# kursawe/OpticalFlow

Hardware: AMD Instinct MI355X
Metric: frame-pairs/sec (higher is better)
Workload: dtype f64; 1 GPU; 1024x1024x256 synthetic translating texture (seed 1), speed_alpha=1, remodelling_alpha=1e4, rtol=1e-06, all 255 pairs solved to the stopping rule; frames_per_gpu=256, pairs_in_flight=255, levels=9, coarse_stencils=float8, vcycle_vectors=coarse_float32, w_cycle_level=1, w_cycle_visits=3, warm_start_stride=3, allgather=False, gather_chunks=1, converged=True

## Files before the change

### opticalflow_amd/csrc/vof_device.hpp

```cpp
#pragma once
#include <hip/hip_runtime.h>
#include <stdint.h>
#include <type_traits>

namespace vof {

constexpr int BX = 64;
constexpr int BY = 4;
constexpr int NT = BX * BY;

struct PairScalars {
    double rho, alpha, omega, beta;
    double bnorm2, rnorm2;
    double tol2;
    int iterations;
    int converged;
    int breakdown;
    int halfstep;
};

struct PairParam {
    double alpha, beta;
    int frame;
    int out;
// ... 151 lines not shown
        blk[1] += scale * (s * P * k.Dy / 2);
        blk[2] += scale * (-s * P / 2);
        blk[3] += scale * (s * P * k.Dy / 2);
        blk[4] += scale * alpha;
        blk[6] += scale * (s * P / 2);
        blk[8] += scale * beta;
    } else if (oi == 0) {
        T s = (T)oj;
        blk[0] += scale * alpha;
        blk[1] += scale * (s * P * k.Dx / 2);
        blk[3] += scale * (s * P * k.Dx / 2);
        blk[4] += scale * (P * (s * k.Dy + P) + alpha);
        blk[5] += scale * (-s * P / 2);
        blk[7] += scale * (s * P / 2);
        blk[8] += scale * beta;
    } else {
        T s = (T)(oi * oj);
        blk[1] += scale * (s * P * P / 4);
        blk[3] += scale * (s * P * P / 4);
    }
}

__host__ __device__ constexpr unsigned raw_block_mask(int oi, int oj) {
    return (oi == 0 && oj == 0) ? 0x1DBu
         : (oj == 0)            ? 0x15Fu
         : (oi == 0)            ? 0x1BBu
                                : 0x00Au;
}

template <typename T, typename KT>
__device__ __forceinline__ void folded_block(const KT& k, T alpha, T beta, int p, int q, int ni, int nj, int oi, int oj, T* blk) {
#pragma unroll
    for (int t = 0; t < 9; ++t) blk[t] = (T)0;
    bool gi = (oi == 1 && p == 0) || (oi == -1 && p == ni - 1);
    bool gj = (oj == 1 && q == 0) || (oj == -1 && q == nj - 1);
    add_raw_block(k, alpha, beta, oi, oj, (T)1, blk);
    if (gi) add_raw_block(k, alpha, beta, -oi, oj, (T)1, blk);
    if (gj) add_raw_block(k, alpha, beta, oi, -oj, (T)1, blk);
    if (gi && gj) add_raw_block(k, alpha, beta, -oi, -oj, (T)2, blk);
}

struct Nbr {
    double u[9], w[9], g[9];
};

template <typename XT>
__device__ __forceinline__ void load_nbr(const XT* __restrict__ x, size_t npts, int ni, int nj, int p, int q,
                                         Nbr& n) {
#pragma unroll
    for (int di = -1; di <= 1; ++di) {
        int tp = p + di;
        bool oi = (tp < 0) || (tp >= ni);
        int fp = fold(tp, ni);
#pragma unroll
        for (int dj = -1; dj <= 1; ++dj) {
            int tq = q + dj;
            bool oj = (tq < 0) || (tq >= nj);
            int fq = fold(tq, nj);
            size_t idx = (size_t)fp * nj + fq;
            double s = (oi && oj) ? 2.0 : 1.0;
            int t = (di + 1) * 3 + (dj + 1);
            n.u[t] = s * (double)x[idx];
            n.w[t] = s * (double)x[npts + idx];
            if (di == 0 || dj == 0) n.g[t] = s * (double)x[2 * npts + idx];
        }
    }
}

__device__ __forceinline__ void offdiag0(const PixCoef& k, double alpha, double beta, const Nbr& n, double& y0,
                                         double& y1, double& y2) {
    const double P = k.P;
    const double hPDx = P * k.Dx / 2, hPDy = P * k.Dy / 2, qPP = P * P / 4, hP = P / 2;
    y0 = (P * (P - k.Dx) + alpha) * n.u[1] + (P * (P + k.Dx) + alpha) * n.u[7] + alpha * (n.u[3] + n.u[5]) +
         hPDx * (n.w[5] - n.w[3]) + hPDy * (n.w[7] - n.w[1]) + qPP * ((n.w[8] - n.w[2]) - (n.w[6] - n.w[0])) +
         hP * (n.g[1] - n.g[7]);
    y1 = (P * (P - k.Dy) + alpha) * n.w[3] + (P * (P + k.Dy) + alpha) * n.w[5] + alpha * (n.w[1] + n.w[7]) +
         hPDy * (n.u[7] - n.u[1]) + hPDx * (n.u[5] - n.u[3]) + qPP * ((n.u[8] - n.u[2]) - (n.u[6] - n.u[0])) +
         hP * (n.g[3] - n.g[5]);
    y2 = beta * (n.g[1] + n.g[7] + n.g[3] + n.g[5]) + hP * (n.u[7] - n.u[1]) + hP * (n.w[5] - n.w[3]);
}

struct Diag0 { double axx, ayy, c, inv; };
struct VDiff0 { double du71, dw71, U4, W4; };
template <bool CORNERS, int ZERO = 0, int DC = 0, int PRE = 0>
__device__ __forceinline__ void gs0_point(const double* im, const Nbr& n, double sUL, double sUR, double sDL, double sDR,
                                          double alpha, double beta, double inv_g, int quirks, double b0, double b1,
                                          double b2, double& u, double& w, double& gm, Diag0* dg = nullptr,
                                          const VDiff0* vd = nullptr) {
#pragma clang fp contract(off)
    const double P = im[4];
    const double Dx = (im[7] - im[1]) * 0.5;
    const double Dy = quirks ? Dx : (im[5] - im[3]) * 0.5;
    const double PP = P * P, PDx = P * Dx, PDy = P * Dy, hP = 0.5 * P;
    const double A1 = PP + alpha, qPP = 0.25 * PP, hPDx = 0.5 * PDx, hPDy = 0.5 * PDy;
    double r0, r1, r2;
    if (ZERO == 1) {
        r0 = b0; r1 = b1; r2 = b2;
    } else if (ZERO == 2) {
        const double du53 = n.u[5] - n.u[3], dw53 = n.w[5] - n.w[3];
        const double y0a = fma(hPDx, dw53, alpha * (n.u[3] + n.u[5]));
        const double y1a = A1 * (n.w[3] + n.w[5]);
        const double y1b = fma(hP, n.g[3] - n.g[5], fma(hPDx, du53, PDy * dw53));
        const double y2 = fma(hP, dw53, beta * (n.g[3] + n.g[5]));
        r0 = b0 - y0a; r1 = b1 - (y1a + y1b); r2 = b2 - y2;
    } else {
        double du71, dw71, W4, U4;
        if (PRE) {
            du71 = vd->du71; dw71 = vd->dw71; U4 = vd->U4; W4 = vd->W4;
        } else {
            du71 = n.u[7] - n.u[1]; dw71 = n.w[7] - n.w[1];
            if (CORNERS) {
                W4 = (sDR * n.w[8] - sUR * n.w[2]) - (sDL * n.w[6] - sUL * n.w[0]);
                U4 = (sDR * n.u[8] - sUR * n.u[2]) - (sDL * n.u[6] - sUL * n.u[0]);
            } else {
                W4 = (n.w[8] - n.w[2]) - (n.w[6] - n.w[0]);
                U4 = (n.u[8] - n.u[2]) - (n.u[6] - n.u[0]);
            }
        }
        if (ZERO == 3) {
            const double y0a = A1 * (n.u[1] + n.u[7]);
            const double y0b = fma(hP, n.g[1] - n.g[7], fma(qPP, W4, fma(hPDy, dw71, PDx * du71)));
            const double y1a = fma(hPDy, du71, alpha * (n.w[1] + n.w[7]));
            const double y1b = qPP * U4;
            const double y2 = fma(hP, du71, beta * (n.g[1] + n.g[7]));
            r0 = b0 - (y0a + y0b); r1 = b1 - (y1a + y1b); r2 = b2 - y2;
        } else {
            const double du53 = n.u[5] - n.u[3], dw53 = n.w[5] - n.w[3];
            const double y0a = fma(hPDx, dw53, fma(alpha, n.u[3] + n.u[5], A1 * (n.u[1] + n.u[7])));
            const double y0b = fma(hP, n.g[1] - n.g[7], fma(qPP, W4, fma(hPDy, dw71, PDx * du71)));
            const double y1a = fma(hPDy, du71, fma(alpha, n.w[1] + n.w[7], A1 * (n.w[3] + n.w[5])));
            const double y1b = fma(hP, n.g[3] - n.g[5], fma(qPP, U4, fma(hPDx, du53, PDy * dw53)));
            const double y2 = fma(hP, du71 + dw53, beta * ((n.g[1] + n.g[7]) + (n.g[3] + n.g[5])));
            r0 = b0 - (y0a + y0b); r1 = b1 - (y1a + y1b); r2 = b2 - y2;
        }
    }
    double axx, ayy, c, inv;
    if (DC == 2) {
        axx = dg->axx; ayy = dg->ayy; c = dg->c; inv = dg->inv;
    } else {
        const double Dxx = fma(-2.0, P, im[7] + im[1]);
        const double Dyy = fma(-2.0, P, im[5] + im[3]);
        const double Dxy = (im[8] - im[6] - im[2] + im[0]) * 0.25;
        const double m4a = -4.0 * alpha;
        axx = fma(P, fma(-2.0, P, Dxx), m4a); ayy = fma(P, fma(-2.0, P, Dyy), m4a); c = P * Dxy;
        const double det = fma(axx, ayy, -(c * c));
        inv = __builtin_amdgcn_rcp(det);
        inv = fma(fma(-det, inv, 1.0), inv, inv);
        inv = fma(fma(-det, inv, 1.0), inv, inv);
        if (DC == 1) { dg->axx = axx; dg->ayy = ayy; dg->c = c; dg->inv = inv; }
    }
    u = fma(r0, ayy, -(c * r1)) * inv;
    w = fma(axx, r1, -(c * r0)) * inv;
    gm = fma(-Dy, w, fma(-Dx, u, r2)) * inv_g;
}

__global__ __launch_bounds__(NT) void k_rhs(const double* __restrict__ frames, size_t frame_stride, int Nj, int ni,
                                            int nj, double* __restrict__ b, const PairParam* __restrict__ pp) {
    int q = blockIdx.x * BX + threadIdx.x, p = blockIdx.y * BY + threadIdx.y, pair = blockIdx.z;
    if (p >= ni || q >= nj) return;
    const double* I = frames + (size_t)(pp ? pp[pair].frame : pair) * frame_stride + (size_t)(p + 1) * Nj + (q + 1);
    const double* J = I + frame_stride;
    double P = I[0];
    double dxt = (J[Nj] - J[-Nj] - I[Nj] + I[-Nj]) / 2;
    double dyt = (J[1] - J[-1] - I[1] + I[-1]) / 2;
    double dt = J[0] - I[0];
    size_t npts = (size_t)ni * nj, idx = (size_t)p * nj + q;
    double* bp = b + (size_t)pair * 3 * npts;
    bp[idx] = -P * dxt;
    bp[npts + idx] = -P * dyt;
    bp[2 * npts + idx] = -dt;
}

__global__ __launch_bounds__(NT) void k_gs0(const double* __restrict__ frames, size_t frame_stride, int Nj, int ni,
                                            int nj, double alpha, double beta, int quirks, double* __restrict__ x,
                                            const double* __restrict__ b, int colour,
                                            const ActiveSet act, const PairParam* __restrict__ pp) {
    int pair = act.pair(blockIdx.z);
    if (!act.on(pair)) return;
    int q = 2 * (blockIdx.x * BX + threadIdx.x) + (colour & 1);
    int p = 2 * (blockIdx.y * BY + threadIdx.y) + (colour >> 1);
    if (p >= ni || q >= nj) return;
    int fidx = pair;
    if (pp) { alpha = pp[pair].alpha; beta = pp[pair].beta; fidx = pp[pair].frame; }
    size_t npts = (size_t)ni * nj, idx = (size_t)p * nj + q, off = (size_t)pair * 3 * npts;
    const double* c = frames + (size_t)fidx * frame_stride + (size_t)(p + 1) * Nj + (q + 1);
    const double im[9] = {c[-Nj - 1], c[-Nj], c[-Nj + 1], c[-1], c[0], c[1], c[Nj - 1], c[Nj], c[Nj + 1]};
    const double* xp = x + off;
    const bool oU = p - 1 < 0, oD = p + 1 >= ni, oL = q - 1 < 0, oR = q + 1 >= nj;
    const size_t rU = (size_t)fold(p - 1, ni) * nj, rC = (size_t)p * nj, rD = (size_t)fold(p + 1, ni) * nj;
    const int qL = fold(q - 1, nj), qR = fold(q + 1, nj);
    Nbr n;
    n.u[0] = xp[rU + qL]; n.w[0] = xp[npts + rU + qL];
    n.u[1] = xp[rU + q];  n.w[1] = xp[npts + rU + q];  n.g[1] = xp[2 * npts + rU + q];
    n.u[2] = xp[rU + qR]; n.w[2] = xp[npts + rU + qR];
    n.u[3] = xp[rC + qL]; n.w[3] = xp[npts + rC + qL]; n.g[3] = xp[2 * npts + rC + qL];
    n.u[5] = xp[rC + qR]; n.w[5] = xp[npts + rC + qR]; n.g[5] = xp[2 * npts + rC + qR];
    n.u[6] = xp[rD + qL]; n.w[6] = xp[npts + rD + qL];
    n.u[7] = xp[rD + q];  n.w[7] = xp[npts + rD + q];  n.g[7] = xp[2 * npts + rD + q];
    n.u[8] = xp[rD + qR]; n.w[8] = xp[npts + rD + qR];
    const double sUL = (oU && oL) ? 2.0 : 1.0, sUR = (oU && oR) ? 2.0 : 1.0;
    const double sDL = (oD && oL) ? 2.0 : 1.0, sDR = (oD && oR) ? 2.0 : 1.0;
    double u, w, g;
    gs0_point<true>(im, n, sUL, sUR, sDL, sDR, alpha, beta, 1.0 / (-1 - 4 * beta), quirks, b[off + idx], b[off + npts + idx],
                    b[off + 2 * npts + idx], u, w, g);
    x[off + idx] = u;
    x[off + npts + idx] = w;
    x[off + 2 * npts + idx] = g;
}

template <typename CT, typename VT>
__device__ __forceinline__ void stencil_offdiag(const CoefSet<CT>& cs, size_t npts, const VT* __restrict__ x,
                                                int ni, int nj, int p, int q, double& y0, double& y1, double& y2,
                                                bool include_diag) {
    y0 = y1 = y2 = 0.0;
#pragma unroll
    for (int a = 0; a < 3; ++a) {
        int tp = p + a - 1;
// ... 2955 lines not shown
```

### opticalflow_amd/csrc/vof_sweep0r.hpp

```cpp
#pragma once
#include "vof_device.hpp"

namespace vof {

__device__ __forceinline__ double lane_shr1(double v) {
    int lo = __double2loint(v), hi = __double2hiint(v);
    lo = __builtin_amdgcn_mov_dpp(lo, 0x138, 0xF, 0xF, true);
    hi = __builtin_amdgcn_mov_dpp(hi, 0x138, 0xF, 0xF, true);
    return __hiloint2double(hi, lo);
}
__device__ __forceinline__ double lane_shl1(double v) {
    int lo = __double2loint(v), hi = __double2hiint(v);
    lo = __builtin_amdgcn_mov_dpp(lo, 0x130, 0xF, 0xF, true);
    hi = __builtin_amdgcn_mov_dpp(hi, 0x130, 0xF, 0xF, true);
    return __hiloint2double(hi, lo);
}

#ifndef VOF_S0R_DCACHE
#define VOF_S0R_DCACHE 1
#endif
#ifndef VOF_S0R_BRING
#define VOF_S0R_BRING 1
#endif
#ifndef VOF_S0R_BL_DC
#define VOF_S0R_BL_DC 1
#endif
#ifndef VOF_S0R_BCARRY
#define VOF_S0R_BCARRY 1
#endif
#ifndef VOF_S0R_FZ_WAVES
#define VOF_S0R_FZ_WAVES 2
#endif
template <int NS, int TRAIL = 0> struct S0R {
    static constexpr int EXT = TRAIL ? 1 : 0;
    static constexpr int LO = 2 * NS + EXT;
    static constexpr int NRW = LO + 4;
    static constexpr int HALO = 4 * NS + 2 * EXT, OUT = S0_W - 2 * HALO;
    static constexpr int IPW = 66;
    static constexpr int IRB = 2 * IPW * 8;
    static constexpr int NRI = LO + 2;
    static constexpr int LDS_BYTES = NRI * IRB;
    static constexpr bool BL = (VOF_S0R_BRING != 0) && NS == 2 && TRAIL == 1;
    static constexpr bool DC = (VOF_S0R_DCACHE != 0) && NS == 2 && (!BL || VOF_S0R_BL_DC);
    static constexpr bool DCT = DC && !BL;
    static constexpr int ND = DC ? 2 * NS + (DCT ? EXT : 0) : 0;
    static constexpr int DRB = 4 * 64 * 16;
    static constexpr int NBL = BL ? 4 : 0, BRB = 3 * 64 * 16;
    static constexpr int LDS_TOTAL = LDS_BYTES + ND * DRB + NBL * BRB;
};

struct S0RRow { double2 u, w, g; };

__device__ __forceinline__ S0RRow round_row32(const S0RRow& s) {
    auto r = [](double2 v) { return double2{(double)(float)v.x, (double)(float)v.y}; };
    return S0RRow{r(s.u), r(s.w), r(s.g)};
}

template <int NS, bool EC, bool FROM_ZERO, int TRAIL, typename ET, int PO, int QK = 1, int BF = 0, typename XT = double>
__global__ __launch_bounds__(64) __attribute__((amdgpu_waves_per_eu((FROM_ZERO && (BF == 0 || BF == 3) && TRAIL != 2) ? VOF_S0R_FZ_WAVES : 1, (FROM_ZERO && (BF == 0 || BF == 3) && TRAIL != 2) ? VOF_S0R_FZ_WAVES : 1))) void k_sweep0r(
    Fine0 pol, int ni, int nj, int TI, int , int nx, int ny, int nz, const XT* __restrict__ x_in,
    XT* __restrict__ x_out, const double* __restrict__ b, const ActiveSet act,
    const ET* __restrict__ ecoarse, int nci, int ncj, S0Trail tr, int skip_first = 0, int skip_count = 0,
    S0BSrc bsrc = S0BSrc{nullptr, nullptr, nullptr, nullptr, nullptr, nullptr}) {
    static_assert(BF == 0 || NS == 2, "b is handed from the first sweep's stages to the second's");
    static_assert(BF == 0 || BF == 3 || (FROM_ZERO && !EC && TRAIL != 1 && PO == 0), "the folded vector update belongs to the first pre-smoothing pass");
    static_assert(TRAIL != 2 || (FROM_ZERO && !EC && PO == 0 && BF != 0), "the residual + restriction stage belongs to the pre-smoothing pass");
    constexpr bool RR = TRAIL == 2;
    static_assert(std::is_same<XT, double>::value || std::is_same<XT, float>::value, "x is stored as float64 or float32");
    constexpr bool X32 = std::is_same<XT, float>::value;
    typedef S0R<NS, TRAIL> G;
    constexpr int W = S0_W, LO = G::LO, NRW = G::NRW, NRI = G::NRI, IRB = G::IRB, IHB = G::IPW * 8, EXT = G::EXT;
    constexpr int NST = 2 * NS, po = PO;
    constexpr bool DC = G::DC;
    constexpr int ND = G::ND, DRB = G::DRB;
    extern __shared__ double sw_lds[];
    char* iring = reinterpret_cast<char*>(sw_lds);
    char* dring = iring + G::LDS_BYTES;
    char* bring = dring + ND * DRB;
    constexpr bool BL = G::BL && BF == 0;
    int bph = 0;
    const unsigned nblocks = (unsigned)nx * ny * nz;
    unsigned lb = blockIdx.x;
    if ((nblocks & 7u) == 0) lb = (lb & 7u) * (nblocks >> 3) + (lb >> 3);
    const int bxl = lb % nx, by = (lb / nx) % ny;
    const int bx = bxl < skip_first ? bxl : bxl + skip_count;
    const int pair = act.pair(lb / (nx * ny));
    if (!act.on(pair)) return;
    const int lane = threadIdx.x;
    const int p0 = by * TI - po;
    const int qs = bx * G::OUT - G::HALO;
    const size_t npts = (size_t)ni * nj, off = (size_t)pair * 3 * npts;
    const XT* xin = FROM_ZERO ? nullptr : x_in + off;
    XT* xout = x_out + off;
    const double* bp = b + off;
    const size_t ncpts = (size_t)nci * ncj;
    const ET* ec = EC ? ecoarse + (size_t)pair * 3 * ncpts : nullptr;
    double alpha = pol.alpha, beta = pol.beta;
    int fidx = pair;
    if (pol.pp) { alpha = pol.pp[pair].alpha; beta = pol.pp[pair].beta; fidx = pol.pp[pair].frame; }
    const double* img = pol.frames + (size_t)fidx * pol.frame_stride;
    const int Nj = pol.Nj;
    constexpr int quirks = QK;
    const double inv_g = 1.0 / (-1 - 4 * beta);

    const int qpair = qs + 2 * lane;
    const bool pair_ok = qpair >= 0 && qpair + 1 < nj;
    const size_t qg = pair_ok ? (size_t)qpair : 0;
    const bool ipair_ok = qpair >= 0 && qpair + 1 <= nj + 1;
    const size_t iqg = ipair_ok ? (size_t)qpair : 0;
    const int xq = qs + 2 * 64;
    const bool xpair_ok = lane == 0 && xq >= 0 && xq + 1 <= nj + 1;
    const bool st_ok = pair_ok && lane >= G::HALO / 2 && lane < (W - G::HALO) / 2;
    const bool glE = qpair == 0, grO = qpair + 1 == nj - 1;
    const bool border_strip = qs < 0 || qs + W > nj;
    const int cqs = qs >> 1;

    S0RRow X[NRW];
#pragma unroll
    for (int j = 0; j < NRW; ++j) X[j].u = X[j].w = X[j].g = double2{0.0, 0.0};
    double2 B[NST][3];
    double2 BV[2][3], BQ[2][3];
    double2 BC[2][2][3];
    double bss = 0.0, bcA = 0.0, bcB = 0.0;
    const double* bfr = nullptr; const double* bfv = nullptr; const double* bfq = nullptr; double* bfo = nullptr;
    if constexpr (BF == 3) bfr = bp;
    if constexpr (BF != 0) {
        if (BF != 3) { bfr = bsrc.r + off; bfv = bsrc.v + off; bfo = bsrc.out + off; }
        if (BF == 1) bcA = bsrc.sc[pair].alpha;
        if (BF == 2) { bfq = bsrc.p_old + off; bcA = bsrc.sc[pair].beta; bcB = bsrc.sc[pair].omega; }
#pragma unroll
        for (int a = 0; a < 2; ++a)
#pragma unroll
            for (int f = 0; f < 3; ++f) { BV[a][f] = BQ[a][f] = BC[0][a][f] = BC[1][a][f] = double2{0.0, 0.0}; }
    }
    double2 li[2] = {{0, 0}, {0, 0}}, lix[2] = {{0, 0}, {0, 0}};
    float2 xf[2][3] = {{{0, 0}, {0, 0}, {0, 0}}, {{0, 0}, {0, 0}, {0, 0}}};
    ET crv[3] = {0, 0, 0};
    double CR[2][3];
    double2 tn[2][3];
    double2 BCo[3];
    double hprev[3] = {0.0, 0.0, 0.0};
    double ts0 = 0.0, ts1 = 0.0;
#pragma unroll
    for (int r = 0; r < 2; ++r)
#pragma unroll
        for (int f = 0; f < 3; ++f) { CR[r][f] = 0.0; tn[r][f] = double2{0.0, 0.0}; BCo[f] = double2{0.0, 0.0}; }

    auto st_lo = [](int st) { const int k = st >> 1, odd = st & 1; return -2 * (NS - 1 - k + EXT) + odd; };
    auto st_hi = [TI](int st) { const int k = st >> 1, odd = st & 1; return TI + 2 * (NS - 1 - k + EXT) - odd; };

    const int s_first = -(NS + EXT) - 1, s_last = (TI + 2 * NS - 2) / 2;
    const int e0 = 2 * s_first;
    int e_lo = 2 * NS, e_hi = TI + 2 * (NS + EXT) - 4;
    e_lo = max(e_lo, 2 * NS - p0);  e_hi = min(e_hi, ni - 4 - p0);
    e_hi = min(e_hi, TI + 2 * NS - 2);
#pragma unroll
    for (int st = 0; st < NST; ++st) {
        e_lo = max(e_lo, max(st_lo(st) + st, 1 - p0 + st));
        e_hi = min(e_hi, min(st_hi(st) + st - 2, ni - 4 - p0 + st));
    }
    if (TRAIL) {
        e_lo = max(e_lo, 2 * NS + 1 - p0);
        e_hi = min(e_hi, min(TI + 2 * NS - 4, ni - 5 - p0 + 2 * NS));
    }
    if (EC) { e_lo = max(e_lo, -p0); e_hi = min(e_hi, 2 * nci - 8 - p0); }

    int islot = 0;
    auto irow = [&](int j) { int s = islot + j; if (s >= NRI) s -= NRI; return iring + s * IRB; };
    int dslot = 0;
    auto drow = [&](int k) { int s = dslot - k; if (s < 0) s += ND; return dring + s * DRB + lane * 16; };

    auto request_rows = [&](auto edge_tag, int e) {
        constexpr bool EDGE = decltype(edge_tag)::value;
        const bool do_load = EDGE ? (e + 3 <= TI + 2 * (NS + EXT) - 1) : true;
#pragma unroll
        for (int r = 0; r < 2; ++r) {
            const int pL = p0 + e + 2 + r;
            if (FROM_ZERO) X[LO + 2 + r].u = X[LO + 2 + r].w = X[LO + 2 + r].g = double2{0.0, 0.0};
            if (!FROM_ZERO && X32) {
                const bool rowok = EDGE ? (do_load && pL >= 0 && pL < ni) : true;
                if (EDGE) xf[r][0] = xf[r][1] = xf[r][2] = float2{0.0f, 0.0f};
                if (EDGE ? (rowok && pair_ok) : true) {
                    const XT* src = xin + (size_t)pL * nj + qg;
#pragma unroll
                    for (int f = 0; f < 3; ++f) xf[r][f] = *reinterpret_cast<const float2*>(src + f * npts);
                }
            } else if (!FROM_ZERO) {
                const bool rowok = EDGE ? (do_load && pL >= 0 && pL < ni) : true;
                S0RRow& d = X[LO + 2 + r];
                if (EDGE) d.u = d.w = d.g = double2{0.0, 0.0};
                if (EDGE ? (rowok && pair_ok) : true) {
                    const XT* src = xin + (size_t)pL * nj + qg;
                    d.u = *reinterpret_cast<const double2*>(src);
                    d.w = *reinterpret_cast<const double2*>(src + npts);
                    d.g = *reinterpret_cast<const double2*>(src + 2 * npts);
                }
            }
            {
                const int pI = pL + 1;
                const bool rowok = EDGE ? (do_load && pI >= 0 && pI <= ni + 1) : true;
                if (EDGE) { li[r] = double2{0.0, 0.0}; lix[r] = double2{0.0, 0.0}; }
                if (rowok) {
                    const double* frow = img + (size_t)pI * Nj;
                    if (EDGE ? ipair_ok : true) li[r] = *reinterpret_cast<const double2*>(frow + iqg);
                    if (EDGE ? xpair_ok : true) lix[r] = *reinterpret_cast<const double2*>(frow + xq);
                }
            }
        }
        if constexpr (EC) {
            const int knew = ((p0 + e + 2) >> 1) + 2;
#pragma unroll
            for (int f = 0; f < 3; ++f) {
                crv[f] = 0;
                const int c0 = cqs + lane;
                if (EDGE ? (knew >= 0 && knew < nci && c0 >= 0 && c0 < ncj) : true) crv[f] = ec[(size_t)f * ncpts + (size_t)knew * ncj + c0];
            }
        }
    };

    auto request_b = [&](auto edge_tag, auto st_tag, int e_next) {
        constexpr bool EDGE = decltype(edge_tag)::value;
        constexpr int st = decltype(st_tag)::value;
        const int rr = e_next - st, p = p0 + rr;
// ... 235 lines not shown
                n.u[4] = RC.u.y; n.w[4] = RC.w.y; n.g[4] = RC.g.y;
                n.u[7] = RD.u.y; n.w[7] = RD.w.y; n.g[7] = RD.g.y;
                n.u[3] = RC.u.x; n.w[3] = RC.w.x; n.g[3] = RC.g.x;
                n.u[5] = lane_shl1(RC.u.x); n.w[5] = lane_shl1(RC.w.x); n.g[5] = lane_shl1(RC.g.x);
                if (VPRE) {
                    vd.du71 = dU.y; vd.dw71 = dW.y;
                    vd.U4 = lane_shl1(dU.x) - dU.x; vd.W4 = lane_shl1(dW.x) - dW.x;
                } else {
                    n.u[0] = RU.u.x; n.w[0] = RU.w.x;
                    n.u[6] = RD.u.x; n.w[6] = RD.w.x;
                    n.u[2] = lane_shl1(RU.u.x); n.w[2] = lane_shl1(RU.w.x);
                    n.u[8] = lane_shl1(RD.u.x); n.w[8] = lane_shl1(RD.w.x);
                }
                if (BORDER && grO) {
                    gr = true;
                    n.u[2] = n.u[0]; n.w[2] = n.w[0]; n.u[5] = n.u[3]; n.w[5] = n.w[3]; n.g[5] = n.g[3]; n.u[8] = n.u[6]; n.w[8] = n.w[6];
                }
                imv[0] = iuB; imv[1] = iuC; imv[2] = iuD; imv[3] = icB; imv[4] = icC; imv[5] = icD; imv[6] = idB; imv[7] = idC; imv[8] = idD;
            }
            double y0, y1, y2;
            Diag0 dg;
            if (par == 0) { dg.axx = dq[0].x; dg.ayy = dq[1].x; dg.c = dq[2].x; }
            else { dg.axx = dq[0].y; dg.ayy = dq[1].y; dg.c = dq[2].y; }
            dg.inv = 0.0;
            if (EDGE) {
                const double sUL = (oU && gl) ? 2.0 : 1.0, sUR = (oU && gr) ? 2.0 : 1.0;
                const double sDL = (oD && gl) ? 2.0 : 1.0, sDR = (oD && gr) ? 2.0 : 1.0;
                apply0_point<true, DCT>(imv, n, sUL, sUR, sDL, sDR, alpha, beta, quirks, y0, y1, y2, &dg);
            } else {
                apply0_point<false, DCT, 1>(imv, n, 1.0, 1.0, 1.0, 1.0, alpha, beta, quirks, y0, y1, y2, &dg, &vd);
            }
            if (par == 0) { y[0].x = y0; y[1].x = y1; y[2].x = y2; }
            else { y[0].y = y0; y[1].y = y1; y[2].y = y2; }
        }
        if constexpr (RR) { yout[0] = y[0]; yout[1] = y[1]; yout[2] = y[2]; return true; }
        if (st_ok) {
            double* vrow = tr.v + off + (size_t)p * nj + qg;
            *reinterpret_cast<double2*>(vrow) = y[0];
            *reinterpret_cast<double2*>(vrow + npts) = y[1];
            *reinterpret_cast<double2*>(vrow + 2 * npts) = y[2];
        }
        const double vv = (y[0].x * y[0].x + y[1].x * y[1].x + y[2].x * y[2].x) + (y[0].y * y[0].y + y[1].y * y[1].y + y[2].y * y[2].y);
        const double vt = (y[0].x * t0.x + y[1].x * t1.x + y[2].x * t2.x) + (y[0].y * t0.y + y[1].y * t1.y + y[2].y * t2.y);
        ts0 += st_ok ? (tr.dotvec ? vt : vv) : 0.0;
        ts1 += st_ok ? vv : 0.0;
        return true;
    };

    auto step = [&](auto edge_tag, auto border_tag, const int e) {
        constexpr bool EDGE = decltype(edge_tag)::value;
        request_rows(edge_tag, e);
        auto run_stage = [&](auto st_tag) {
            constexpr int ST = decltype(st_tag)::value;
            const int rr = e - ST, p = p0 + rr;
            const bool rowok = EDGE ? (rr >= st_lo(ST) && rr <= st_hi(ST) && p >= 0 && p < ni) : true;
            if constexpr (BF != 0 && ST < 2) {
                double2 bs[3];
#pragma unroll
                for (int f = 0; f < 3; ++f) {
                    if (BF == 3) {
                        bs[f] = B[ST][f];
                    } else if (BF == 1) {
                        bs[f].x = fma(-bcA, BV[ST][f].x, B[ST][f].x);
                        bs[f].y = fma(-bcA, BV[ST][f].y, B[ST][f].y);
                    } else {
                        bs[f].x = fma(bcA, fma(-bcB, BV[ST][f].x, BQ[ST][f].x), B[ST][f].x);
                        bs[f].y = fma(bcA, fma(-bcB, BV[ST][f].y, BQ[ST][f].y), B[ST][f].y);
                    }
                    BC[1][ST][f] = bs[f];
                }
                const bool own = st_ok && rr >= 0 && rr < TI && p < ni;
                if (BF != 3 && own) {
                    double* orow = bfo + (size_t)p * nj + qg;
                    *reinterpret_cast<double2*>(orow) = bs[0];
                    *reinterpret_cast<double2*>(orow + npts) = bs[1];
                    *reinterpret_cast<double2*>(orow + 2 * npts) = bs[2];
                }
                if (BF == 1) {
                    const double q = (bs[0].x * bs[0].x + bs[0].y * bs[0].y) + (bs[1].x * bs[1].x + bs[1].y * bs[1].y) + (bs[2].x * bs[2].x + bs[2].y * bs[2].y);
                    bss += own ? q : 0.0;
                }
                if (rowok) stage(edge_tag, border_tag, std::integral_constant<int, LO - ST>{}, rr, bs);
            } else if constexpr (BF != 0) {
                if (rowok) stage(edge_tag, border_tag, std::integral_constant<int, LO - ST>{}, rr, BC[0][ST - 2]);
            } else if constexpr (BL && ST < 2) {
                if (rowok) stage(edge_tag, border_tag, std::integral_constant<int, LO - ST>{}, rr, B[ST]);
                char* bw = bring + (ST * 2 + bph) * G::BRB + lane * 16;
#pragma unroll
                for (int f = 0; f < 3; ++f) *reinterpret_cast<double2*>(bw + f * 1024) = B[ST][f];
            } else if constexpr (BL) {
                double2 bl[3];
                const char* br = bring + ((ST - 2) * 2 + (bph ^ 1)) * G::BRB + lane * 16;
#pragma unroll
                for (int f = 0; f < 3; ++f) bl[f] = *reinterpret_cast<const double2*>(br + f * 1024);
                if (rowok) stage(edge_tag, border_tag, std::integral_constant<int, LO - ST>{}, rr, bl);
            } else {
                if (rowok) stage(edge_tag, border_tag, std::integral_constant<int, LO - ST>{}, rr, B[ST]);
            }
            request_b(edge_tag, st_tag, e + 2);
        };
        run_stage(std::integral_constant<int, 0>{});
        run_stage(std::integral_constant<int, 1>{});
        if constexpr (NST > 2) {
            run_stage(std::integral_constant<int, 2>{});
            run_stage(std::integral_constant<int, 3>{});
        }
        if constexpr (X32 && TRAIL != 0) {
            X[LO - 2 * NS] = round_row32(X[LO - 2 * NS]);
            X[LO - 2 * NS + 1] = round_row32(X[LO - 2 * NS + 1]);
        }
        if constexpr (TRAIL == 1) {
            double2 yd[3];
            trail_row(edge_tag, border_tag, std::integral_constant<int, LO - 2 * NS + 1>{}, e - 2 * NS + 1, std::integral_constant<int, 1>{}, yd);
            trail_row(edge_tag, border_tag, std::integral_constant<int, LO - 2 * NS>{}, e - 2 * NS, std::integral_constant<int, 0>{}, yd);
        }
        if constexpr (RR) {
            double2 ya[3], yb[3];
            const bool okb = trail_row(edge_tag, border_tag, std::integral_constant<int, LO - 2 * NS + 1>{}, e - 2 * NS + 1, std::integral_constant<int, 1>{}, yb);
            const bool oka = trail_row(edge_tag, border_tag, std::integral_constant<int, LO - 2 * NS>{}, e - 2 * NS, std::integral_constant<int, 0>{}, ya);
            const int rrA = e - 2 * NS, pA = p0 + rrA, cp = pA >> 1;
            const int cq = (qs >> 1) + lane;
            const double wR = (EDGE && cq + 1 >= ncj) ? 1.0 : 0.5;
            const double wD = (EDGE && cp + 1 >= nci) ? 1.0 : 0.5;
            double cv[3];
#pragma unroll
            for (int f = 0; f < 3; ++f) {
                double2 ra = {0.0, 0.0}, rb = {0.0, 0.0};
                if (EDGE ? (oka && pair_ok) : true) { ra.x = BCo[f].x - ya[f].x; ra.y = BCo[f].y - ya[f].y; }
                if (EDGE ? (okb && pair_ok) : true) { rb.x = BC[0][1][f].x - yb[f].x; rb.y = BC[0][1][f].y - yb[f].y; }
                const double ha = fma(0.5, lane_shr1(ra.y), fma(wR, ra.y, ra.x));
                const double hb = fma(0.5, lane_shr1(rb.y), fma(wR, rb.y, rb.x));
                cv[f] = 0.25 * fma(0.5, hprev[f], fma(wD, hb, ha));
                hprev[f] = hb;
            }
            const bool own = st_ok && rrA >= 0 && rrA < TI && pA < ni && (EDGE ? (cq < ncj && cp < nci) : true);
            if (own) {
                ET* bc = reinterpret_cast<ET*>(tr.v) + (size_t)pair * 3 * ncpts + (size_t)cp * ncj + cq;
                bc[0] = (ET)cv[0]; bc[ncpts] = (ET)cv[1]; bc[2 * ncpts] = (ET)cv[2];
            }
#pragma unroll
            for (int f = 0; f < 3; ++f) BCo[f] = BC[0][0][f];
        }
#pragma unroll
        for (int r = 0; r < 2; ++r) {
            const int rrW = e - 2 * NS + r, pW = p0 + rrW;
            const bool rowok = EDGE ? (rrW >= 0 && rrW < TI && pW >= 0 && pW < ni) : true;
            if (rowok && st_ok) {
                const S0RRow& s = X[LO - 2 * NS + r];
                XT* dst = xout + (size_t)pW * nj + qg;
                if constexpr (X32) {
                    *reinterpret_cast<float2*>(dst) = float2{(float)s.u.x, (float)s.u.y};
                    *reinterpret_cast<float2*>(dst + npts) = float2{(float)s.w.x, (float)s.w.y};
                    *reinterpret_cast<float2*>(dst + 2 * npts) = float2{(float)s.g.x, (float)s.g.y};
                } else {
                    *reinterpret_cast<double2*>(dst) = s.u;
                    *reinterpret_cast<double2*>(dst + npts) = s.w;
                    *reinterpret_cast<double2*>(dst + 2 * npts) = s.g;
                }
            }
        }
        {
            const bool do_load = EDGE ? (e + 3 <= TI + 2 * (NS + EXT) - 1) : true;
            if (do_load) {
#pragma unroll
                for (int r = 0; r < 2; ++r) {
                    char* dst = irow(r);
                    *reinterpret_cast<double*>(dst + lane * 8) = li[r].x;
                    *reinterpret_cast<double*>(dst + IHB + lane * 8) = li[r].y;
                    if (EDGE ? lane == 0 : true) {
                        *reinterpret_cast<double*>(dst + 64 * 8) = lix[r].x;
                        *reinterpret_cast<double*>(dst + IHB + 64 * 8) = lix[r].y;
                    }
                }
            }
            islot += 2;
            if (islot >= NRI) islot -= NRI;
            if (DC) { dslot += 2; if (dslot >= ND) dslot -= ND; }
            if (BL) bph ^= 1;
            __builtin_amdgcn_fence(__ATOMIC_RELEASE, "wavefront");
            __builtin_amdgcn_wave_barrier();
        }
        if constexpr (X32 && !FROM_ZERO) {
#pragma unroll
            for (int r = 0; r < 2; ++r) {
                S0RRow& d = X[LO + 2 + r];
                d.u = double2{(double)xf[r][0].x, (double)xf[r][0].y};
                d.w = double2{(double)xf[r][1].x, (double)xf[r][1].y};
                d.g = double2{(double)xf[r][2].x, (double)xf[r][2].y};
            }
        }
        if constexpr (EC) {
            const int pL0 = p0 + e + 2;
            double cnew[3];
#pragma unroll
            for (int f = 0; f < 3; ++f) cnew[f] = (double)crv[f];
#pragma unroll
            for (int r = 0; r < 2; ++r) {
                const int pL = pL0 + r;
                const bool rowok = EDGE ? (e + 3 <= TI + 2 * (NS + EXT) - 1 && pL >= 0 && pL < ni) : true;
// ... 77 lines not shown
```

Baseline: 1415 frame-pairs/s.

## Compute fused residual-restriction from sweep deltas instead of re-evaluating full stencil

New measurement: 1400 frame-pairs/s. 0.989x the previous value.

```diff
diff --git a/opticalflow_amd/csrc/vof_device.hpp b/opticalflow_amd/csrc/vof_device.hpp
--- a/opticalflow_amd/csrc/vof_device.hpp
+++ b/opticalflow_amd/csrc/vof_device.hpp
@@ -257,27 +257,22 @@
 
 struct Diag0 { double axx, ayy, c, inv; };
 struct VDiff0 { double du71, dw71, U4, W4; };
-template <bool CORNERS, int ZERO = 0, int DC = 0, int PRE = 0>
-__device__ __forceinline__ void gs0_point(const double* im, const Nbr& n, double sUL, double sUR, double sDL, double sDR,
-                                          double alpha, double beta, double inv_g, int quirks, double b0, double b1,
-                                          double b2, double& u, double& w, double& gm, Diag0* dg = nullptr,
-                                          const VDiff0* vd = nullptr) {
+
+template <bool CORNERS, int ZERO, int PRE>
+__device__ __forceinline__ void offdiag0_sums(double P, double Dx, double Dy, const Nbr& n, double sUL, double sUR, double sDL,
+                                              double sDR, double alpha, double beta, const VDiff0* vd, double& y0, double& y1,
+                                              double& y2) {
 #pragma clang fp contract(off)
-    const double P = im[4];
-    const double Dx = (im[7] - im[1]) * 0.5;
-    const double Dy = quirks ? Dx : (im[5] - im[3]) * 0.5;
+    static_assert(ZERO == 0 || ZERO == 2 || ZERO == 3, "ZERO = 1 has no off-diagonal part");
     const double PP = P * P, PDx = P * Dx, PDy = P * Dy, hP = 0.5 * P;
     const double A1 = PP + alpha, qPP = 0.25 * PP, hPDx = 0.5 * PDx, hPDy = 0.5 * PDy;
-    double r0, r1, r2;
-    if (ZERO == 1) {
-        r0 = b0; r1 = b1; r2 = b2;
-    } else if (ZERO == 2) {
+    if (ZERO == 2) {
         const double du53 = n.u[5] - n.u[3], dw53 = n.w[5] - n.w[3];
         const double y0a = fma(hPDx, dw53, alpha * (n.u[3] + n.u[5]));
         const double y1a = A1 * (n.w[3] + n.w[5]);
         const double y1b = fma(hP, n.g[3] - n.g[5], fma(hPDx, du53, PDy * dw53));
-        const double y2 = fma(hP, dw53, beta * (n.g[3] + n.g[5]));
-        r0 = b0 - y0a; r1 = b1 - (y1a + y1b); r2 = b2 - y2;
+        y0 = y0a; y1 = y1a + y1b;
+        y2 = fma(hP, dw53, beta * (n.g[3] + n.g[5]));
     } else {
         double du71, dw71, W4, U4;
         if (PRE) {
@@ -297,17 +292,36 @@
             const double y0b = fma(hP, n.g[1] - n.g[7], fma(qPP, W4, fma(hPDy, dw71, PDx * du71)));
             const double y1a = fma(hPDy, du71, alpha * (n.w[1] + n.w[7]));
             const double y1b = qPP * U4;
-            const double y2 = fma(hP, du71, beta * (n.g[1] + n.g[7]));
-            r0 = b0 - (y0a + y0b); r1 = b1 - (y1a + y1b); r2 = b2 - y2;
+            y0 = y0a + y0b; y1 = y1a + y1b;
+            y2 = fma(hP, du71, beta * (n.g[1] + n.g[7]));
         } else {
             const double du53 = n.u[5] - n.u[3], dw53 = n.w[5] - n.w[3];
             const double y0a = fma(hPDx, dw53, fma(alpha, n.u[3] + n.u[5], A1 * (n.u[1] + n.u[7])));
             const double y0b = fma(hP, n.g[1] - n.g[7], fma(qPP, W4, fma(hPDy, dw71, PDx * du71)));
             const double y1a = fma(hPDy, du71, fma(alpha, n.w[1] + n.w[7], A1 * (n.w[3] + n.w[5])));
             const double y1b = fma(hP, n.g[3] - n.g[5], fma(qPP, U4, fma(hPDx, du53, PDy * dw53)));
-            const double y2 = fma(hP, du71 + dw53, beta * ((n.g[1] + n.g[7]) + (n.g[3] + n.g[5])));
-            r0 = b0 - (y0a + y0b); r1 = b1 - (y1a + y1b); r2 = b2 - y2;
-        }
+            y0 = y0a + y0b; y1 = y1a + y1b;
+            y2 = fma(hP, du71 + dw53, beta * ((n.g[1] + n.g[7]) + (n.g[3] + n.g[5])));
+        }
+    }
+}
+
+template <bool CORNERS, int ZERO = 0, int DC = 0, int PRE = 0>
+__device__ __forceinline__ void gs0_point(const double* im, const Nbr& n, double sUL, double sUR, double sDL, double sDR,
+                                          double alpha, double beta, double inv_g, int quirks, double b0, double b1,
+                                          double b2, double& u, double& w, double& gm, Diag0* dg = nullptr,
+                                          const VDiff0* vd = nullptr) {
+#pragma clang fp contract(off)
+    const double P = im[4];
+    const double Dx = (im[7] - im[1]) * 0.5;
+    const double Dy = quirks ? Dx : (im[5] - im[3]) * 0.5;
+    double r0, r1, r2;
+    if (ZERO == 1) {
+        r0 = b0; r1 = b1; r2 = b2;
+    } else {
+        double y0, y1, y2;
+        offdiag0_sums<CORNERS, ZERO == 1 ? 0 : ZERO, PRE>(P, Dx, Dy, n, sUL, sUR, sDL, sDR, alpha, beta, vd, y0, y1, y2);
+        r0 = b0 - y0; r1 = b1 - y1; r2 = b2 - y2;
     }
     double axx, ayy, c, inv;
     if (DC == 2) {
diff --git a/opticalflow_amd/csrc/vof_sweep0r.hpp b/opticalflow_amd/csrc/vof_sweep0r.hpp
--- a/opticalflow_amd/csrc/vof_sweep0r.hpp
+++ b/opticalflow_amd/csrc/vof_sweep0r.hpp
@@ -31,9 +31,14 @@
 #ifndef VOF_S0R_FZ_WAVES
 #define VOF_S0R_FZ_WAVES 2
 #endif
+#ifndef VOF_S0R_RR_DELTA
+#define VOF_S0R_RR_DELTA 1
+#endif
 template <int NS, int TRAIL = 0> struct S0R {
     static constexpr int EXT = TRAIL ? 1 : 0;
-    static constexpr int LO = 2 * NS + EXT;
+    static constexpr bool RRD = (VOF_S0R_RR_DELTA != 0) && TRAIL == 2;
+    static constexpr int WEXT = RRD ? 0 : EXT;
+    static constexpr int LO = 2 * NS + WEXT;
     static constexpr int NRW = LO + 4;
     static constexpr int HALO = 4 * NS + 2 * EXT, OUT = S0_W - 2 * HALO;
     static constexpr int IPW = 66;
@@ -42,7 +47,7 @@
     static constexpr int LDS_BYTES = NRI * IRB;
     static constexpr bool BL = (VOF_S0R_BRING != 0) && NS == 2 && TRAIL == 1;
     static constexpr bool DC = (VOF_S0R_DCACHE != 0) && NS == 2 && (!BL || VOF_S0R_BL_DC);
-    static constexpr bool DCT = DC && !BL;
+    static constexpr bool DCT = DC && !BL && !RRD;
     static constexpr int ND = DC ? 2 * NS + (DCT ? EXT : 0) : 0;
     static constexpr int DRB = 4 * 64 * 16;
     static constexpr int NBL = BL ? 4 : 0, BRB = 3 * 64 * 16;
@@ -65,7 +70,7 @@
     static_assert(BF == 0 || NS == 2, "b is handed from the first sweep's stages to the second's");
     static_assert(BF == 0 || BF == 3 || (FROM_ZERO && !EC && TRAIL != 1 && PO == 0), "the folded vector update belongs to the first pre-smoothing pass");
     static_assert(TRAIL != 2 || (FROM_ZERO && !EC && PO == 0 && BF != 0), "the residual + restriction stage belongs to the pre-smoothing pass");
-    constexpr bool RR = TRAIL == 2;
+    constexpr bool RR = TRAIL == 2, RRD = S0R<NS, TRAIL>::RRD;
     static_assert(std::is_same<XT, double>::value || std::is_same<XT, float>::value, "x is stored as float64 or float32");
     constexpr bool X32 = std::is_same<XT, float>::value;
     typedef S0R<NS, TRAIL> G;
@@ -139,6 +144,10 @@
     double CR[2][3];
     double2 tn[2][3];
     double2 BCo[3];
+    S0RRow D5, D3;
+    double D4y[3] = {0.0, 0.0, 0.0}, D2y[3] = {0.0, 0.0, 0.0};
+    double2 P4 = {0.0, 0.0}, Dx4 = {0.0, 0.0}, Dy4 = {0.0, 0.0};
+    D5.u = D5.w = D5.g = D3.u = D3.w = D3.g = double2{0.0, 0.0};
     double hprev[3] = {0.0, 0.0, 0.0};
     double ts0 = 0.0, ts1 = 0.0;
 #pragma unroll
@@ -540,7 +549,18 @@
                 }
                 if (rowok) stage(edge_tag, border_tag, std::integral_constant<int, LO - ST>{}, rr, bs);
             } else if constexpr (BF != 0) {
+                const S0RRow xo = X[LO - ST];
                 if (rowok) stage(edge_tag, border_tag, std::integral_constant<int, LO - ST>{}, rr, BC[0][ST - 2]);
+                if constexpr (RRD) {
+                    const S0RRow& xn = X[LO - ST];
+                    if (ST == 2) {
+                        D2y[0] = xn.u.y - xo.u.y; D2y[1] = xn.w.y - xo.w.y; D2y[2] = xn.g.y - xo.g.y;
+                    } else {
+                        D3.u.x = xn.u.x - xo.u.x; D3.u.y = xn.u.y - xo.u.y;
+                        D3.w.x = xn.w.x - xo.w.x; D3.w.y = xn.w.y - xo.w.y;
+                        D3.g.x = xn.g.x - xo.g.x; D3.g.y = xn.g.y - xo.g.y;
+                    }
+                }
             } else if constexpr (BL && ST < 2) {
                 if (rowok) stage(edge_tag, border_tag, std::integral_constant<int, LO - ST>{}, rr, B[ST]);
                 char* bw = bring + (ST * 2 + bph) * G::BRB + lane * 16;
@@ -563,7 +583,7 @@
             run_stage(std::integral_constant<int, 2>{});
             run_stage(std::integral_constant<int, 3>{});
         }
-        if constexpr (X32 && TRAIL != 0) {
+        if constexpr (X32 && TRAIL != 0 && !RRD) {
             X[LO - 2 * NS] = round_row32(X[LO - 2 * NS]);
             X[LO - 2 * NS + 1] = round_row32(X[LO - 2 * NS + 1]);
         }
@@ -572,7 +592,115 @@
             trail_row(edge_tag, border_tag, std::integral_constant<int, LO - 2 * NS + 1>{}, e - 2 * NS + 1, std::integral_constant<int, 1>{}, yd);
             trail_row(edge_tag, border_tag, std::integral_constant<int, LO - 2 * NS>{}, e - 2 * NS, std::integral_constant<int, 0>{}, yd);
         }
-        if constexpr (RR) {
+        if constexpr (RRD) {
+            const int rrA = e - 2 * NS, pA = p0 + rrA, cp = pA >> 1;
+            const bool oka = EDGE ? (rrA >= -1 && rrA < TI && pA >= 0 && pA < ni) : true;
+            const bool okb = EDGE ? (rrA + 1 >= -1 && rrA + 1 < TI && pA + 1 >= 0 && pA + 1 < ni) : true;
+            const bool oU = EDGE && pA - 1 < 0, oD = EDGE && pA + 1 >= ni;
+            S0RRow RU = D5, RD = D3;
+            if (EDGE) {
+                if (oU) RU = D3;
+                if (oD) RD = D5;
+            }
+            constexpr int VPRE = EDGE ? 0 : 1;
+            double2 dU = {0.0, 0.0}, dW = {0.0, 0.0};
+            if (VPRE) {
+                dU.x = RD.u.x - RU.u.x; dU.y = RD.u.y - RU.u.y;
+                dW.x = RD.w.x - RU.w.x; dW.y = RD.w.y - RU.w.y;
+            }
+            double2 ya[3];
+            double yb[3];
+            {
+                Nbr n = {};
+                VDiff0 vd = {0.0, 0.0, 0.0, 0.0};
+                bool gl = false;
+                n.u[1] = RU.u.x; n.w[1] = RU.w.x; n.g[1] = RU.g.x;
+                n.u[7] = RD.u.x; n.w[7] = RD.w.x; n.g[7] = RD.g.x;
+                n.u[5] = D4y[0]; n.w[5] = D4y[1]; n.g[5] = D4y[2];
+                n.u[3] = lane_shr1(D4y[0]); n.w[3] = lane_shr1(D4y[1]); n.g[3] = lane_shr1(D4y[2]);
+                if (VPRE) {
+                    vd.du71 = dU.x; vd.dw71 = dW.x;
+                    vd.U4 = dU.y - lane_shr1(dU.y); vd.W4 = dW.y - lane_shr1(dW.y);
+                } else {
+                    n.u[2] = RU.u.y; n.w[2] = RU.w.y;
+                    n.u[8] = RD.u.y; n.w[8] = RD.w.y;
+                    n.u[0] = lane_shr1(RU.u.y); n.w[0] = lane_shr1(RU.w.y);
+                    n.u[6] = lane_shr1(RD.u.y); n.w[6] = lane_shr1(RD.w.y);
+                }
+                if (decltype(border_tag)::value && glE) {
+                    gl = true;
+                    n.u[0] = n.u[2]; n.w[0] = n.w[2]; n.u[3] = n.u[5]; n.w[3] = n.w[5]; n.g[3] = n.g[5]; n.u[6] = n.u[8]; n.w[6] = n.w[8];
+                }
+                const double sUL = (oU && gl) ? 2.0 : 1.0, sDL = (oD && gl) ? 2.0 : 1.0;
+                offdiag0_sums<EDGE, 0, VPRE>(P4.x, Dx4.x, Dy4.x, n, sUL, 1.0, sDL, 1.0, alpha, beta, &vd, ya[0].x, ya[1].x, ya[2].x);
+            }
+            {
+                Nbr n = {};
+                VDiff0 vd = {0.0, 0.0, 0.0, 0.0};
+                bool gr = false;
+                n.u[1] = RU.u.y; n.w[1] = RU.w.y; n.g[1] = RU.g.y;
+                n.u[7] = RD.u.y; n.w[7] = RD.w.y; n.g[7] = RD.g.y;
+                if (VPRE) {
+                    vd.du71 = dU.y; vd.dw71 = dW.y;
+                    vd.U4 = lane_shl1(dU.x) - dU.x; vd.W4 = lane_shl1(dW.x) - dW.x;
+                } else {
+                    n.u[0] = RU.u.x; n.w[0] = RU.w.x;
+                    n.u[6] = RD.u.x; n.w[6] = RD.w.x;
+                    n.u[2] = lane_shl1(RU.u.x); n.w[2] = lane_shl1(RU.w.x);
+                    n.u[8] = lane_shl1(RD.u.x); n.w[8] = lane_shl1(RD.w.x);
+                }
+                if (decltype(border_tag)::value && grO) {
+                    gr = true;
+                    n.u[2] = n.u[0]; n.w[2] = n.w[0]; n.u[8] = n.u[6]; n.w[8] = n.w[6];
+                }
+                const double sUR = (oU && gr) ? 2.0 : 1.0, sDR = (oD && gr) ? 2.0 : 1.0;
+                offdiag0_sums<EDGE, 3, VPRE>(P4.y, Dx4.y, Dy4.y, n, 1.0, sUR, 1.0, sDR, alpha, beta, &vd, ya[0].y, ya[1].y, ya[2].y);
+            }
+            auto row_pd = [&](auto jc_tag, double2& P, double2& Dx, double2& Dy) {
+                constexpr int jc = decltype(jc_tag)::value;
+                const char* iu = irow(jc - 1);
+                const char* ic = irow(jc);
+                const char* id = irow(jc + 1);
+                auto LD = [](const char* r, int o) { return *reinterpret_cast<const double*>(r + o); };
+                const int ie = lane * 8, io = IHB + lane * 8;
+                P.x = LD(ic, io); P.y = LD(ic, ie + 8);
+                Dx.x = (LD(id, io) - LD(iu, io)) * 0.5; Dx.y = (LD(id, ie + 8) - LD(iu, ie + 8)) * 0.5;
+                Dy.x = quirks ? Dx.x : (LD(ic, ie + 8) - LD(ic, ie)) * 0.5;
+                Dy.y = quirks ? Dx.y : (LD(ic, io + 8) - LD(ic, io)) * 0.5;
+            };
+            {
+                double2 P3, Dx3, Dy3;
+                row_pd(std::integral_constant<int, LO - 2 * NS + 1>{}, P3, Dx3, Dy3);
+                Nbr n = {};
+                n.u[5] = D3.u.y; n.w[5] = D3.w.y; n.g[5] = D3.g.y;
+                n.u[3] = lane_shr1(D3.u.y); n.w[3] = lane_shr1(D3.w.y); n.g[3] = lane_shr1(D3.g.y);
+                if (decltype(border_tag)::value && glE) { n.u[3] = n.u[5]; n.w[3] = n.w[5]; n.g[3] = n.g[5]; }
+                offdiag0_sums<EDGE, 2, 0>(P3.x, Dx3.x, Dy3.x, n, 1.0, 1.0, 1.0, 1.0, alpha, beta, nullptr, yb[0], yb[1], yb[2]);
+            }
+            row_pd(std::integral_constant<int, LO - 2 * NS + 2>{}, P4, Dx4, Dy4);
+            const int cq = (qs >> 1) + lane;
+            const double wR = (EDGE && cq + 1 >= ncj) ? 1.0 : 0.5;
+            const double wD = (EDGE && cp + 1 >= nci) ? 1.0 : 0.5;
+            double cv[3];
+#pragma unroll
+            for (int f = 0; f < 3; ++f) {
+                double2 ma = {0.0, 0.0};
+                double mb = 0.0;
+                if (EDGE ? (oka && pair_ok) : true) ma = ya[f];
+                if (EDGE ? (okb && pair_ok) : true) mb = yb[f];
+                const double ha = fma(0.5, lane_shr1(ma.y), fma(wR, ma.y, ma.x));
+                cv[f] = -0.25 * fma(0.5, hprev[f], fma(wD, mb, ha));
+                hprev[f] = mb;
+            }
+            const bool own = st_ok && rrA >= 0 && rrA < TI && pA < ni && (EDGE ? (cq < ncj && cp < nci) : true);
+            if (own) {
+                ET* bc = reinterpret_cast<ET*>(tr.v) + (size_t)pair * 3 * ncpts + (size_t)cp * ncj + cq;
+                bc[0] = (ET)cv[0]; bc[ncpts] = (ET)cv[1]; bc[2 * ncpts] = (ET)cv[2];
+            }
+            D5 = D3;
+#pragma unroll
+            for (int f = 0; f < 3; ++f) D4y[f] = D2y[f];
+        } else if constexpr (RR) {
             double2 ya[3], yb[3];
             const bool okb = trail_row(edge_tag, border_tag, std::integral_constant<int, LO - 2 * NS + 1>{}, e - 2 * NS + 1, std::integral_constant<int, 1>{}, yb);
             const bool oka = trail_row(edge_tag, border_tag, std::integral_constant<int, LO - 2 * NS>{}, e - 2 * NS, std::integral_constant<int, 0>{}, ya);
diff --git a/profiles/sweep0r_launches.py b/profiles/sweep0r_launches.py
--- /dev/null
+++ b/profiles/sweep0r_launches.py
@@ -0,0 +1,45 @@
+#!/usr/bin/env python3
+import csv
+import re
+import sys
+from collections import defaultdict
+from statistics import median
+
+
+def short(name):
+    return re.sub(r"\(.*", "", name).replace("void ", "").replace("vof::", "").strip()
+
+
+def main():
+    path = sys.argv[1]
+    want = sys.argv[2] if len(sys.argv) > 2 else "k_sweep0r<2, false, true, 2,"
+    total = 0.0
+    by = defaultdict(list)
+    cls = defaultdict(float)
+    with open(path) as f:
+        for r in csv.DictReader(f):
+            us = (int(r["End_Timestamp"]) - int(r["Start_Timestamp"])) / 1e3
+            total += us
+            name = short(r["Kernel_Name"])
+            cls[name.split("<")[0]] += us
+            if want in name:
+                grid = int(r["Grid_Size_X"]) * int(r.get("Grid_Size_Y", 1) or 1) * int(r.get("Grid_Size_Z", 1) or 1)
+                by[(name, grid)].append(us)
+    print(f"all kernels: {total / 1e3:.1f} ms")
+    for k, v in sorted(cls.items(), key=lambda kv: -kv[1])[:8]:
+        print(f"  {k}: {v / 1e3:.1f} ms ({100 * v / total:.1f} %)")
+    sel = sum(sum(v) for v in by.values())
+    print(f"selected: {sum(len(v) for v in by.values())} launches, {sel / 1e3:.1f} ms = {100 * sel / total:.1f} % of the summed kernel time")
+    print("\n| instantiation | grid (threads) | launches | total, us | median, us | min .. max, us |\n|---|---:|---:|---:|---:|---:|")
+    for (name, grid), v in sorted(by.items(), key=lambda kv: (kv[0][0], -kv[0][1])):
+        print(f"| `{name}` | {grid} | {len(v)} | {sum(v):.1f} | {median(v):.1f} | {min(v):.1f} .. {max(v):.1f} |")
+    print("\n| instantiation | launches | total, us |\n|---|---:|---:|")
+    per = defaultdict(list)
+    for (name, _), v in by.items():
+        per[name] += v
+    for name, v in sorted(per.items()):
+        print(f"| `{name}` | {len(v)} | {sum(v):.1f} |")
+
+
+if __name__ == "__main__":
+    main()
```
